# hyye/lio-mapping

Measured on NVIDIA H100. Metric: scans/sec + GN-iter ms, HDL-64 window=10 at 1/2/4/8 H100 vs CPU Ceres ref, higher is better.
Workload: dtype f32 features / f64 solve

## Files before the change

### include/lio_b200.h

```cpp
#ifndef LIO_B200_H_
#define LIO_B200_H_

#include <stddef.h>
#include <stdint.h>

#ifdef __cplusplus
extern "C" {
#endif

typedef enum lio_status {
  LIO_OK = 0,
  LIO_ERR_CUDA = -1,
  LIO_ERR_INVALID = -2,
  LIO_ERR_CAPACITY = -3,
  LIO_ERR_NO_DEVICE = -4,
  LIO_ERR_NUMERIC = -5
} lio_status;

const char *lio_last_error(void);
int lio_version(void);
int lio_device_count(void);

typedef struct lio_pp_config {
  float lower_bound;
// ... 190 lines not shown
int lio_est_set_scan_clouds_dev(lio_est *est, const float *corner_dev, const int *nc_dev, int nc_max, const float *full_dev,
                                const int *nf_dev, int nf_max);
int lio_est_local_clouds_dev(lio_est *est, const float *ptr[3], const int **n_dev, int n_host[3]);
int lio_est_local_clouds_download(lio_est *est, int which, float *out, int cap, int *n);
int lio_est_local_laser_odom(lio_est *est, float tf7[7]);
int lio_est_attach_map(lio_est *est, lio_pm *pm);
int lio_est_map_poses(lio_est *est, float tobe7[7], float aft7[7], float insert7[7], int info4[4]);
int lio_est_get_states(lio_est *est, double *out);
int lio_est_summary(lio_est *est, double *out32);
int lio_est_feature_count(lio_est *est, int frame, int *n);
int lio_est_get_features(lio_est *est, int frame, float *pts4, float *coef4, int32_t *src, int cap);
int lio_est_map_size(lio_est *est, int *n);
int lio_est_get_map(lio_est *est, float *out, int cap);
int lio_est_frame_size(lio_est *est, int frame, int *n);
int lio_est_get_frame(lio_est *est, int frame, float *out, int cap);
int lio_est_get_local_transform(lio_est *est, int frame, float tf7[7]);
int lio_est_prior_dim(lio_est *est, int *n);
int lio_est_get_prior(lio_est *est, double *Hp, double *bp);
int lio_est_last_normal_equations(lio_est *est, double *H, double *g, double *cost, int *n);
int lio_est_last_launches(lio_est *est);
const char *lio_est_last_error(lio_est *est);
int lio_est_solver_trace(lio_est *est, long long *out, int cap);
int lio_est_kernel_profile(lio_est *est, double out[8], int reset);
typedef int (*lio_allreduce_fn)(void *user, double *buf_dev, int count);
int lio_est_set_shard(lio_est *est, int rank, int world, lio_allreduce_fn fn, void *user);
int lio_est_exchange_buffer(lio_est *est, void **dev_ptr, size_t *bytes);
int lio_est_set_peers(lio_est *est, int world, void *const *peer_ptrs );
int lio_est_feature_slab(lio_est *est, void **dev_ptr, size_t *bytes);
int lio_est_set_feature_peers(lio_est *est, int world, void *const *peer_slabs );
int lio_ipc_export(const void *dev_ptr, unsigned char handle[64]);
int lio_ipc_open(const unsigned char handle[64], void **dev_ptr);
int lio_ipc_close(void *dev_ptr);
int lio_est_frame_owner(int frame_rel, int world);

int lio_compact_encode(const float tf7[7], const float *corner, int nc, const float *surf, int ns, const float *full, int nf,
                       float *out_xyzi, int cap_points, int *n_points);
int lio_compact_sizes(const float *xyzi, int n_points, int sizes[3]);
int lio_compact_decode(const float *xyzi, int n_points, float tf7[7], float *corner, float *surf, float *full);
int lio_xyzi_to_pcl32(const float *xyzi, int n, uint8_t *out32);
int lio_pcl32_to_xyzi(const uint8_t *in32, int n, float *xyzi);

int lio_host_cholesky_solve(int n, const double *A, const double *b, double *L_out, double *x);
int lio_host_sym_eigen(int n, const double *A, double *evals, double *evecs, int threads);
int lio_host_dogleg_toy(int n, int m, const double *A, const double *B, const double *y, double amp, int use_cauchy, double *x,
                        int max_iter, double *summary);

// ... 5 lines not shown
```

### lio_mapping_b200/_lib.py

```python
from __future__ import annotations

import ctypes as C
import os

import numpy as np

_HERE = os.path.dirname(os.path.abspath(__file__))
LIB_PATH = os.path.join(_HERE, "liblio_b200.so")
_LIB = None


class LioError(RuntimeError):
    pass


STATUS = {0: "LIO_OK", -1: "LIO_ERR_CUDA", -2: "LIO_ERR_INVALID", -3: "LIO_ERR_CAPACITY", -4: "LIO_ERR_NO_DEVICE",
          -5: "LIO_ERR_NUMERIC"}

f32p = np.ctypeslib.ndpointer(np.float32, flags="C_CONTIGUOUS")
f64p = np.ctypeslib.ndpointer(np.float64, flags="C_CONTIGUOUS")
i32p = np.ctypeslib.ndpointer(np.int32, flags="C_CONTIGUOUS")
u8p = np.ctypeslib.ndpointer(np.uint8, flags="C_CONTIGUOUS")
i8p = np.ctypeslib.ndpointer(np.int8, flags="C_CONTIGUOUS")

# ... 128 lines not shown
    L.lio_ipc_export.argtypes = [vp, u8p]
    L.lio_ipc_open.argtypes = [u8p, C.POINTER(vp)]
    L.lio_ipc_close.argtypes = [vp]
    L.lio_est_process_imu_batch.argtypes = [vp, ip, f64p, f64p, f64p, f64p]
    L.lio_est_process_scan_dev.argtypes = [vp, vp, vp, ip]
    L.lio_est_get_states.argtypes = [vp, f64p]
    L.lio_est_summary.argtypes = [vp, f64p]
    L.lio_est_feature_count.argtypes = [vp, ip, C.POINTER(ip)]
    L.lio_est_get_features.argtypes = [vp, ip, f32p, f32p, i32p, ip]
    L.lio_est_map_size.argtypes = [vp, C.POINTER(ip)]
    L.lio_est_get_map.argtypes = [vp, f32p, ip]
    L.lio_est_frame_size.argtypes = [vp, ip, C.POINTER(ip)]
    L.lio_est_get_frame.argtypes = [vp, ip, f32p, ip]
    L.lio_est_get_local_transform.argtypes = [vp, ip, f32p]
    L.lio_est_prior_dim.argtypes = [vp, C.POINTER(ip)]
    L.lio_est_get_prior.argtypes = [vp, f64p, f64p]
    L.lio_est_last_normal_equations.argtypes = [vp, f64p, f64p, C.POINTER(C.c_double), C.POINTER(ip)]
    L.lio_est_last_launches.argtypes = [vp]
    L.lio_est_last_error.argtypes = [vp]
    L.lio_est_last_error.restype = C.c_char_p
    L.lio_est_solver_trace.argtypes = [vp, np.ctypeslib.ndpointer(np.int64, flags="C_CONTIGUOUS"), ip]
    L.lio_est_frame_owner.argtypes = [ip, ip]
    L.lio_est_kernel_profile.argtypes = [vp, f64p, ip]
    L.lio_est_set_shard.argtypes = [vp, ip, ip, ALLREDUCE_FN, vp]
    L.lio_est_enable_local_clouds.argtypes = [vp, C.c_float, ip, ip]
    L.lio_est_set_scan_clouds_host.argtypes = [vp, f32p, ip, f32p, ip]
    L.lio_est_set_scan_clouds_dev.argtypes = [vp, vp, vp, ip, vp, vp, ip]
    L.lio_est_local_clouds_dev.argtypes = [vp, C.POINTER(vp), C.POINTER(vp), i32p]
    L.lio_est_local_clouds_download.argtypes = [vp, ip, f32p, ip, C.POINTER(ip)]
    L.lio_est_local_laser_odom.argtypes = [vp, f32p]
    L.lio_est_attach_map.argtypes = [vp, vp]
    L.lio_est_map_poses.argtypes = [vp, f32p, f32p, f32p, i32p]
    L.lio_mb_process_map_dev.argtypes = [vp, vp, vp, vp, vp, i32p, f32p, f32p, f32p, i32p]
    L.lio_po_process_dev.argtypes = [vp, C.POINTER(vp), C.POINTER(vp), i32p, f32p, f32p, i32p]
    L.lio_po_clouds_dev.argtypes = [vp, C.POINTER(vp), C.POINTER(vp), i32p]
    L.lio_pm_process_dev.argtypes = [vp, vp, vp, vp, vp, i32p, f32p, f32p, f32p, i32p]
    L.lio_pm_enable_publish.argtypes = [vp, C.c_float, ip]
    L.lio_pm_update_map_database_host.argtypes = [vp, f32p, ip, f32p, ip, np.ctypeslib.ndpointer(np.int64, flags="C_CONTIGUOUS"), ip,
                                                  f32p, i32p]
    L.lio_pm_update_stats.argtypes = [vp, i32p]
    _LIB = L
    return L


def check(rc: int, what: str = ""):
    if rc != 0:
# ... 10 lines not shown
```

### lio_mapping_b200/csrc/estimator.cu

```cuda
#include "assemble.cuh"
#include "cubemap.cuh"
#include <atomic>
#include <condition_variable>
#include <functional>
#include <mutex>
#include <thread>
#include "factors_host.h"
#include "factors_impl.h"
#include "knn.cuh"
#include "odom.cuh"
#include "qr.cuh"
#include "solver_dev.cuh"
#include "solver_host.h"
#include "voxel.cuh"
#include <chrono>
#include <cstddef>
#include <memory>
#include <new>
#include <vector>

namespace lio {
using namespace hm;

constexpr int kMaxWindow = 32;
// ... 269 lines not shown
      st->AtA[a * 6 + b] = v; st->AtA[b * 6 + a] = v;
    } else {
      st->AtB[threadIdx.x - 21] = v;
    }
  }
  __syncthreads();
  if (threadIdx.x == 0) odom_solve_step(st, tf_dev, delta_r_abort, delta_t_abort);
}

}

using namespace lio;
using namespace lio::hm;

struct lio_pim {
  std::shared_ptr<Preintegration> p;
};

struct ImuStampedF {
  double time;
  float q[4];
  float p[3];
};

struct MargPrior {
  bool valid = false;
  int n = 0;
  Mat Hp;
  Vec bp;
  double c0 = 0;
  std::vector<double> x0_pose, x0_sb;
  double x0_ex[7];
};

constexpr size_t kXRowBytes = sizeof(double) * kMaxOpt * kAsmStride;
constexpr size_t kXFlagOff = 2 * kXRowBytes;
constexpr size_t kXErrOff = kXFlagOff + sizeof(unsigned) * kMaxPeers;
constexpr size_t kXBytes = kXErrOff + 64;

struct MargJob {
  bool stashed = false, running = false;
  int O = 0;
  Mat A;
  Vec b;
  std::vector<double> x0_pose, x0_sb;
  double x0_ex[7];
// ... 172 lines not shown
  bool frames_started = false;
  float lc_corner_leaf = 0.2f;
  int lc_cap[2] = {0, 0};
  std::vector<float4 *> lc_slot[2];
  int *d_lc_slot_n = nullptr;
  float4 *d_lc_stage[2] = {nullptr, nullptr};
  int *d_lc_stage_n = nullptr;
  float4 *d_lc_pub[3] = {nullptr, nullptr, nullptr};
  int *d_lc_pub_n = nullptr;
  int lc_pub_cap[3] = {0, 0, 0};
  VoxelGrid lc_vg;
  cudaStream_t lc_stream = nullptr;
  cudaEvent_t lc_ev_fork = nullptr, lc_ev_join = nullptr;
  TransformF es{0, 0, 0, 1, 0, 0, 0};
  lio_pm *map = nullptr;
  bool scanned = false;
  int map_scans = 0;
  bool map_pending = false;
  float4 *d_keep[2] = {nullptr, nullptr};
  int *d_keep_n = nullptr;
  cudaEvent_t map_ev_in = nullptr, map_ev_done = nullptr;
  lio::TwistF map_insert;
  int map_info[4] = {0, 0, 0, 0};
};

static Tw tlb_double(const lio_est *e) {
  return Tw(Q(e->tlb_q[3], e->tlb_q[0], e->tlb_q[1], e->tlb_q[2]), V3(e->tlb_p[0], e->tlb_p[1], e->tlb_p[2]));
}

static Tw lidar_pose(const V3 &P, const M3 &R, const Tw &tlb) {
  Q rot = fromR(R * toR(inverse(tlb.rot)));
  V3 pos = P - rotate(rot, tlb.pos);
  return Tw(rot, pos);
}

struct AffineF { float R[9]; float t[3]; TransformF tf; };
static AffineF to_affine_f(const Tw &t) {
  AffineF a;
  float qx = (float)t.rot.x, qy = (float)t.rot.y, qz = (float)t.rot.z, qw = (float)t.rot.w;
  float n = std::sqrt(qx * qx + qy * qy + qz * qz + qw * qw);
  qx /= n; qy /= n; qz /= n; qw /= n;
  const float tx = 2.f * qx, ty = 2.f * qy, tz = 2.f * qz;
  const float twx = tx * qw, twy = ty * qw, twz = tz * qw, txx = tx * qx, txy = ty * qx, txz = tz * qx;
  const float tyy = ty * qy, tyz = tz * qy, tzz = tz * qz;
  a.R[0] = 1.f - (tyy + tzz); a.R[1] = txy - twz; a.R[2] = txz + twy;
  a.R[3] = txy + twz; a.R[4] = 1.f - (txx + tzz); a.R[5] = tyz - twx;
  a.R[6] = txz - twy; a.R[7] = tyz + twx; a.R[8] = 1.f - (txx + tyy);
// ... 108 lines not shown
  if (e->xbuf) cudaFree(e->xbuf);
  if (e->h_tf) cudaFreeHost(e->h_tf);
  if (e->h_S) cudaFreeHost(e->h_S);
  if (e->h_Rt) cudaFreeHost(e->h_Rt);
  if (e->d_Rt) cudaFree(e->d_Rt);
  if (e->h_counts) cudaFreeHost(e->h_counts);
  e->vg.destroy(); e->hash.destroy(); e->knn.destroy(); e->knn2.destroy(); e->asmw.destroy();
  if (e->ostream) cudaStreamDestroy(e->ostream);
  if (e->ev_map) cudaEventDestroy(e->ev_map);
  if (e->ev_odom) cudaEventDestroy(e->ev_odom);
  if (e->lc_stream) cudaStreamSynchronize(e->lc_stream);
  for (int w = 0; w < 2; ++w) {
    for (float4 *p : e->lc_slot[w]) if (p) cudaFree(p);
    if (e->d_lc_stage[w]) cudaFree(e->d_lc_stage[w]);
  }
  for (int w = 0; w < 3; ++w) if (e->d_lc_pub[w]) cudaFree(e->d_lc_pub[w]);
  if (e->d_lc_slot_n) cudaFree(e->d_lc_slot_n);
  if (e->d_lc_stage_n) cudaFree(e->d_lc_stage_n);
  if (e->d_lc_pub_n) cudaFree(e->d_lc_pub_n);
  e->lc_vg.destroy();
  if (e->lc_stream) cudaStreamDestroy(e->lc_stream);
  if (e->lc_ev_fork) cudaEventDestroy(e->lc_ev_fork);
  if (e->lc_ev_join) cudaEventDestroy(e->lc_ev_join);
  delete e;
  return LIO_OK;
}

extern "C" int lio_est_create(const lio_est_config *cfg, int device, void *cuda_stream, lio_est **out) {
  if (!cfg || !out) return LIO_ERR_INVALID;
  const int W = cfg->window_size, O = cfg->opt_window_size;
  if (W < 1 || W >= kMaxWindow || O < 1 || O > W || O > kMaxOpt || cfg->max_frame_points < 16 || cfg->max_scan_points < 16 ||
      !(cfg->surf_filter_size > 0) || !(cfg->min_match_sq_dis > 0) || cfg->odom_max_iterations < 1) {
    lio_set_last_error(__FILE__, __LINE__, "lio_est_create: configuration outside supported limits");
    return LIO_ERR_INVALID;
  }
  if (lio_device_count() <= 0) return LIO_ERR_NO_DEVICE;
  LIO_CUDA_OK(cudaSetDevice(device));
  lio_est *e = new (std::nothrow) lio_est();
  if (!e) return LIO_ERR_INVALID;
  e->cfg = *cfg; e->W = W; e->O = O; e->device = device; e->stream = (cudaStream_t)cuda_stream;
  cudaDeviceGetAttribute(&e->sm_count, cudaDevAttrMultiProcessorCount, device);
  e->noise.acc_n = cfg->acc_n; e->noise.gyr_n = cfg->gyr_n; e->noise.acc_w = cfg->acc_w; e->noise.gyr_w = cfg->gyr_w; e->noise.g_norm = cfg->g_norm;
  e->g_vec = V3(0, 0, -cfg->g_norm);
  e->extrinsic_stage = cfg->estimate_extrinsic;
  e->Ps.assign(W + 1, V3()); e->Vs.assign(W + 1, V3()); e->Bas.assign(W + 1, V3()); e->Bgs.assign(W + 1, V3());
  e->Rs.assign(W + 1, M3::I());
// ... 15 lines not shown
  }
  e->local_cap = e->slot_cap + cfg->max_frame_points * (O > 1 ? O - 1 : 1);
  ok = ok && cudaMalloc(&e->d_slot_n, sizeof(int) * (W + 1)) == cudaSuccess;
  ok = ok && cudaMalloc(&e->d_own_n, sizeof(int) * (W + 1)) == cudaSuccess;
  ok = ok && cudaMalloc(&e->d_scan, sizeof(float4) * cfg->max_scan_points) == cudaSuccess;
  ok = ok && cudaMalloc(&e->d_local, sizeof(float4) * e->local_cap) == cudaSuccess;
  ok = ok && cudaMalloc(&e->d_map, sizeof(float4) * e->local_cap) == cudaSuccess;
  ok = ok && cudaMalloc(&e->d_tmp, sizeof(float4) * e->slot_cap) == cudaSuccess;
  ok = ok && cudaMalloc(&e->d_counts, sizeof(int) * 8) == cudaSuccess;
  ok = ok && cudaMalloc(&e->d_tf, sizeof(TransformF) * (W + 1)) == cudaSuccess;
  ok = ok && cudaMalloc(&e->d_odom, sizeof(OdomState)) == cudaSuccess;
  ok = ok && cudaMalloc(&e->d_odom_partial, sizeof(double) * 32 * 1024) == cudaSuccess;
  ok = ok && cudaMallocHost((void **)&e->h_tf, sizeof(TransformF) * (W + 1)) == cudaSuccess;
  ok = ok && cudaMallocHost((void **)&e->h_S, sizeof(double) * kMaxOpt * kAsmStride) == cudaSuccess;
  ok = ok && cudaMallocHost((void **)&e->h_Rt, sizeof(double) * kMaxOpt * kAsmRtStride) == cudaSuccess;
  ok = ok && cudaMalloc(&e->d_Rt, sizeof(double) * kMaxOpt * kAsmRtStride) == cudaSuccess;
  ok = ok && cudaMallocHost((void **)&e->h_counts, sizeof(int) * (W + 16)) == cudaSuccess;
  if (ok) { std::memset(e->h_counts, 0, sizeof(int) * (W + 16)); e->h_xerr = e->h_counts + W + 10; }
  int vg_cap = std::max(e->local_cap, cfg->max_scan_points);
  ok = ok && e->vg.init(vg_cap) == 0;
  ok = ok && e->hash.init(e->local_cap) == 0;
  ok = ok && e->knn.init(cfg->max_frame_points * (O + 1)) == 0;
  ok = ok && e->knn2.init(cfg->max_frame_points) == 0;
  ok = ok && cudaStreamCreateWithFlags(&e->ostream, cudaStreamNonBlocking) == cudaSuccess;
  ok = ok && cudaEventCreateWithFlags(&e->ev_map, cudaEventDisableTiming) == cudaSuccess;
  ok = ok && cudaEventCreateWithFlags(&e->ev_odom, cudaEventDisableTiming) == cudaSuccess;
  e->feats.assign(W + 1, FeatureOut());
  long long total_feat = 0;
  {
    e->foff_pts.assign(W + 1, 0); e->foff_coef.assign(W + 1, 0);
    size_t off = 0;
    for (int k = pivot + 1; k <= W; ++k) {
      const int cap = cfg->max_frame_points * ((k == W && cfg->keep_features) ? cfg->odom_max_iterations : 1);
      e->feats[k].cap = cap;
      e->foff_pts[k] = off; off += sizeof(float4) * (size_t)cap;
      e->foff_coef[k] = off; off += sizeof(float4) * (size_t)cap;
      total_feat += cap;
    }
    e->foff_cnt = off; off += ((sizeof(int) * (size_t)(W + 1) + 255) / 256) * 256;
    e->fpar_stride = off;
    e->foff_flags = 2 * off;
    e->fslab_bytes = 2 * off + 256;
    ok = ok && cudaMalloc(&e->fslab, e->fslab_bytes) == cudaSuccess && cudaMemset(e->fslab, 0, e->fslab_bytes) == cudaSuccess;
    for (int k = pivot + 1; k <= W && ok; ++k) ok = ok && cudaMalloc(&e->feats[k].src, sizeof(int) * e->feats[k].cap) == cudaSuccess;
    if (ok) set_feature_parity(e, 0);
  }
  ok = ok && e->asmw.init((int)std::min<long long>(total_feat, 1ll << 30)) == 0;
// ... 342 lines not shown
  for (int i = 0; i <= W; ++i) {
    AffineF a = to_affine_f(tw_mul(pivot_inv, lidar_pose(e->Ps[i], e->Rs[i], tlb)));
    e->local_tf[i] = a.tf;
    e->h_tf[i] = a.tf;
    if (i < pivot || i == W) continue;
    cp.src[ns] = e->slot_ptr[e->slot_of[i]];
    cp.n[ns] = e->d_slot_n + e->slot_of[i];
    if (i == pivot) cp.identity[ns] = 1;
    else { std::memcpy(cp.R[ns], a.R, sizeof(a.R)); std::memcpy(cp.t[ns], a.t, sizeof(a.t)); cp.tag[ns] = (float)i; }
    ++ns;
  }
  cp.nsrc = ns;
  EST_CUDA(cudaMemcpyAsync(e->d_tf, e->h_tf, sizeof(TransformF) * (W + 1), cudaMemcpyHostToDevice, st));
  k_concat<<<std::max(1, std::min(e->sm_count * 4, (e->local_cap + 255) / 256)), 256, 0, st>>>(cp, e->d_local, e->d_counts + 1, e->local_cap);
  ++e->launches;
  long long bound = 64;
  for (int i = 0; i < W; ++i) bound += e->size_surf_stack[i] > 0 ? e->size_surf_stack[i] : e->cfg.max_frame_points;
  const int n_bound = (int)std::min<long long>(e->local_cap, bound);
  int rc = e->vg.run(e->d_local, e->d_counts + 1, n_bound, e->cfg.surf_filter_size, e->d_map, e->local_cap, e->d_counts + 2, nullptr, st, &e->launches);
  if (rc != LIO_OK) return rc;
  const float cell = std::sqrt(e->cfg.min_match_sq_dis) * (1.0f + 1.0f / 1024.0f);
  rc = e->hash.build(e->d_map, e->d_counts + 2, n_bound, cell, st, &e->launches);
  if (rc != LIO_OK) return rc;
  e->t_build = now_s() - t0;
  const double t1 = now_s();
  if (e->fpeers) {
    set_feature_parity(e, e->fparity ^ 1);
    ++e->fepoch;
    for (int idx = pivot + 1; idx <= W; ++idx)
      if (owns_frame(e, idx)) EST_CUDA(cudaMemsetAsync(e->d_feat_counts + idx, 0, sizeof(int), st));
  } else {
    EST_CUDA(cudaMemsetAsync(e->d_feat_counts, 0, sizeof(int) * (W + 1), st));
  }
  constexpr int kOdomFirstBatch = 3;
  const bool odom = e->cfg.imu_factor && owns_frame(e, W);
  KnnBatch ob;
  auto odom_rounds = [&](int from, int to, cudaStream_t q) -> int {
    const int idx = W, slot = e->slot_of[W];
    if (!e->cfg.keep_features) {
      ob.nframes = 1;
      KnnFrame &f = ob.f[0];
      f.surf = e->slot_ptr[slot]; f.n_dev = e->d_slot_n + slot; f.n_bound = e->cfg.max_frame_points; f.tf = e->d_tf + idx;
      f.out_p = e->feats[idx].pts; f.out_c = e->feats[idx].coef; f.out_src = e->feats[idx].src; f.out_count = e->feats[idx].count;
      f.append = 0; f.tile0 = 0;
      for (int it = from; it < to; ++it) {
        int r2 = calculate_features_batch(e->hash, ob, e->cfg.min_match_sq_dis, e->cfg.min_plane_dis, &e->d_odom->done, e->knn2, q, &e->launches,
// ... 26 lines not shown
    rc = odom_rounds(0, odom_first, e->ostream);
    if (rc != LIO_OK) return rc;
    EST_CUDA(cudaEventRecord(e->ev_odom, e->ostream));
  }
  {
    KnnBatch b;
    b.nframes = 0;
    for (int idx = pivot + 1; idx <= W; ++idx) {
      if (!owns_frame(e, idx)) continue;
      if (idx == W && e->cfg.imu_factor) continue;
      const int slot = e->slot_of[idx];
      KnnFrame &f = b.f[b.nframes++];
      f.surf = e->slot_ptr[slot]; f.n_dev = e->d_slot_n + slot; f.tf = e->d_tf + idx;
      const int known = e->size_surf_stack[idx];
      f.n_bound = (known > 0 && idx < W) ? known : e->cfg.max_frame_points;
      f.out_p = e->feats[idx].pts; f.out_c = e->feats[idx].coef; f.out_src = e->feats[idx].src; f.out_count = e->feats[idx].count;
      f.append = 0; f.tile0 = 0;
    }
    e->knn_timed = b.nframes > 0 && e->evk0 && e->evk1;
    if (e->knn_timed) cudaEventRecord(e->evk0, st);
    rc = calculate_features_batch(e->hash, b, e->cfg.min_match_sq_dis, e->cfg.min_plane_dis, nullptr, e->knn, st, &e->launches);
    if (rc != LIO_OK) return rc;
    if (e->knn_timed) cudaEventRecord(e->evk1, st);
  }
  auto readback = [&]() -> int {
    EST_CUDA(cudaMemcpyAsync(e->h_counts, e->d_feat_counts, sizeof(int) * (W + 1), cudaMemcpyDeviceToHost, st));
    EST_CUDA(cudaMemcpyAsync(e->h_counts + W + 1, e->d_counts, sizeof(int) * 4, cudaMemcpyDeviceToHost, st));
    EST_CUDA(cudaMemcpyAsync(e->h_counts + W + 5, &e->d_odom->iter, sizeof(int), cudaMemcpyDeviceToHost, st));
    EST_CUDA(cudaMemcpyAsync(e->h_tf + W, e->d_tf + W, sizeof(TransformF), cudaMemcpyDeviceToHost, st));
    EST_CUDA(cudaMemcpyAsync(e->h_counts + W + 6, e->d_slot_n + e->slot_of[W], sizeof(int), cudaMemcpyDeviceToHost, st));
    EST_CUDA(cudaMemcpyAsync(e->h_counts + W + 7, e->vg.overflow_flag(), sizeof(int), cudaMemcpyDeviceToHost, st));
    EST_CUDA(cudaMemcpyAsync(e->h_counts + W + 8, &e->d_odom->done, sizeof(int), cudaMemcpyDeviceToHost, st));
    if (e->fpeers) EST_CUDA(cudaMemcpyAsync(e->h_counts + W + 9, e->fslab + e->foff_flags + 128, sizeof(int), cudaMemcpyDeviceToHost, st));
    if (e->map) EST_CUDA(cudaMemcpyAsync(e->h_counts + W + 13, e->d_lc_stage_n + 1, sizeof(int), cudaMemcpyDeviceToHost, st));
    EST_CUDA(cudaStreamSynchronize(st));
    return LIO_OK;
  };
  if (odom) EST_CUDA(cudaStreamWaitEvent(st, e->ev_odom, 0));
  if (e->fpeers) {
    const size_t pbase = (size_t)e->fparity * e->fpar_stride;
    FeaturePeers fp;
    std::memset(&fp, 0, sizeof(fp));
    fp.npeers = e->world; fp.self = e->rank;
    FlagPeers fl;
    std::memset(&fl, 0, sizeof(fl));
    fl.npeers = e->world; fl.self = e->rank;
    for (int r = 0; r < e->world; ++r) fl.flag[r] = reinterpret_cast<unsigned *>(e->fpeer_base[r] + e->foff_flags);
    for (int idx = pivot + 1; idx <= W; ++idx) {
      if (!owns_frame(e, idx)) continue;
      for (int r = 0; r < e->world; ++r) {
        fp.pts[r] = reinterpret_cast<float4 *>(e->fpeer_base[r] + pbase + e->foff_pts[idx]);
        fp.coef[r] = reinterpret_cast<float4 *>(e->fpeer_base[r] + pbase + e->foff_coef[idx]);
        fp.count[r] = reinterpret_cast<int *>(e->fpeer_base[r] + pbase + e->foff_cnt) + idx;
      }
      const int known = e->size_surf_stack[idx];
      const int bound = (known > 0 && idx < W) ? known : e->feats[idx].cap;
      k_publish_features<<<std::max(1, std::min(e->sm_count * 2, (bound + 255) / 256)), 256, 0, st>>>(e->feats[idx].pts, e->feats[idx].coef, e->feats[idx].count,
                                                                                                   e->feats[idx].cap, fp);
      ++e->launches;
    }
    k_publish_flag<<<1, 32, 0, st>>>(fl, e->fepoch);
    k_xwait<<<1, 32, 0, st>>>(reinterpret_cast<const unsigned *>(e->fslab + e->foff_flags), e->world, e->fepoch,
                              reinterpret_cast<int *>(e->fslab + e->foff_flags + 128), nullptr);
    e->launches += 2;
  }
  if (before_sync) {
    rc = before_sync();
    if (rc != LIO_OK) return rc;
  }
  rc = readback();
  if (rc != LIO_OK) return rc;
  if (odom && odom_first < odom_total && !e->h_counts[W + 8]) {
    rc = odom_rounds(odom_first, odom_total, st);
    if (rc != LIO_OK) return rc;
    rc = readback();
    if (rc != LIO_OK) return rc;
  }
  if (e->fpeers && (rc = xwait_report(e, Exchange::features, st)) != LIO_OK) return rc;
  if (e->h_counts[W + 6] > e->cfg.max_frame_points) {
    lio_set_last_error(__FILE__, __LINE__, "down-sampled scan exceeds max_frame_points");
    return LIO_ERR_CAPACITY;
  }
  if (e->h_counts[W + 7]) {
    cudaMemsetAsync(e->vg.overflow_flag(), 0, sizeof(int), st);
    lio_set_last_error(__FILE__, __LINE__, "voxel grid index overflow (leaf size too small for the cloud extent)");
    return LIO_ERR_CAPACITY;
  }
  e->size_surf_stack[W] = e->h_counts[W + 6];
  if (e->knn_timed) {
    float ms = 0.f;
    if (cudaEventElapsedTime(&ms, e->evk0, e->evk1) == cudaSuccess) {
      long long nq = 0;
      for (int idx = pivot + 1; idx <= W; ++idx)
        if (owns_frame(e, idx) && !(idx == W && e->cfg.imu_factor)) nq += e->size_surf_stack[idx];
      e->knn_ms_sum += ms; e->knn_launch_count += 1; e->knn_query_sum += nq;
    }
  }
  for (int k = 0; k <= W; ++k) e->h_feat_n[k] = e->h_counts[k];
  e->h_map_n = e->h_counts[W + 1 + 2];
  e->odom_iters = e->h_counts[W + 5];
// ... 303 lines not shown
      add_lidar_block(S, ft[i].M, &H, &g, off_pose(0), off_pose(i), oe);
    }
    e->t_lin_lidar += now_s() - tl0;
  }
  cost = cp + ci + cm + cprior;
  if (c_pim) *c_pim = ci;
  if (c_ppp) *c_ppp = cp;
  if (c_marg) *c_marg = cm;
  return std::isfinite(cost) ? LIO_OK : LIO_ERR_NUMERIC;
}

static void prior_join(lio_est *e);
static int solve_dev_prepare(lio_est *e, int max_it, bool assemble_only);
static int slide_window(lio_est *e);
static MargPrior marg_algebra(Mat A, Vec b, int O, std::vector<double> x0_pose, std::vector<double> x0_sb, const double *x0_ex);
static int marginalize(lio_est *e) {
  const int O = e->O, pivot = e->W - O;
  const int m = 15, nr = 15 * O + 6, pos = m + nr;
  Mat A(pos, pos);
  Vec b(pos, 0.0);
  auto idx_pose = [&](int k) { return k == 0 ? 0 : m + 15 * (k - 1); };
  auto idx_sb = [&](int k) { return k == 0 ? 6 : m + 15 * (k - 1) + 6; };
  const int idx_ex = m + 15 * O;
  if (e->prior.valid) {
    const MargPrior &pr = e->prior;
    Vec dx;
    prior_dx(e, pr, dx);
    Vec Hdx;
    matvec(pr.Hp, dx, Hdx);
    auto map = [&](int pi) {
      if (pi >= 15 * O) return idx_ex + (pi - 15 * O);
      int k = pi / 15, a = pi % 15;
      return (a < 6 ? idx_pose(k) + a : idx_sb(k) + (a - 6));
    };
    for (int a = 0; a < pr.n; ++a) {
      const int ia = map(a);
      b[ia] += Hdx[a] + pr.bp[a];
      for (int c = 0; c < pr.n; ++c) A(ia, map(c)) += pr.Hp(a, c);
    }
  }
  if (e->cfg.imu_factor && e->pre[pivot + 1]->sum_dt < 10.0) {
    double r[15], J[15][30];
    imu_factor_evaluate30(*e->pre[pivot + 1], e->para_pose[0].data(), e->para_sb[0].data(), e->para_pose[1].data(), e->para_sb[1].data(), r, J);
    int col[30];
    for (int c = 0; c < 6; ++c) { col[c] = idx_pose(0) + c; col[15 + c] = idx_pose(1) + c; }
    for (int c = 0; c < 9; ++c) { col[6 + c] = idx_sb(0) + c; col[21 + c] = idx_sb(1) + c; }
    add_JtJ_mapped(&J[0][0], r, 15, 30, col, A, b);
  }
  if (e->cfg.point_distance_factor) {
    std::vector<FrameTerms> ft;
    int rc = eval_lidar(e, ft);
    if (rc != LIO_OK) return rc;
    for (int i = 1; i <= O; ++i) add_lidar_block(e->h_S + (i - 1) * kAsmStride, ft[i].M, &A, &b, idx_pose(0), idx_pose(i), idx_ex);
  }
  MargJob &job = e->mjob;
  job.O = O;
  job.A.r = A.r; job.A.c = A.c; job.A.d.swap(A.d);
  job.b.swap(b);
  job.x0_pose.resize(7 * O); job.x0_sb.resize(9 * O);
  for (int k = 1; k <= O; ++k) {
    std::memcpy(&job.x0_pose[7 * (k - 1)], e->para_pose[k].data(), 7 * sizeof(double));
    std::memcpy(&job.x0_sb[9 * (k - 1)], e->para_sb[k].data(), 9 * sizeof(double));
  }
  std::memcpy(job.x0_ex, e->para_ex, sizeof(job.x0_ex));
  job.stashed = true;
  if (!e->cfg.overlap_marginalization) {
    job.stashed = false;
    e->prior = marg_algebra(std::move(job.A), std::move(job.b), job.O, std::move(job.x0_pose), std::move(job.x0_sb), job.x0_ex);
    e->hp_exp_valid = false;
  }
  return LIO_OK;
}

static MargPrior marg_algebra(Mat A, Vec b, int O, std::vector<double> x0_pose, std::vector<double> x0_sb, const double *x0_ex) {
  const int m = 15, nr = 15 * O + 6;
  const double eps = 1e-8;
  Mat Amm(m, m);
  for (int r = 0; r < m; ++r) for (int c = 0; c < m; ++c) Amm(r, c) = 0.5 * (A(r, c) + A(c, r));
  Vec ev;
  Mat evec;
  sym_eigen(Amm, ev, evec);
  Mat Amm_inv(m, m);
  for (int r = 0; r < m; ++r)
    for (int c = 0; c < m; ++c) { double s = 0; for (int k = 0; k < m; ++k) s += evec(r, k) * (ev[k] > eps ? 1.0 / ev[k] : 0.0) * evec(c, k); Amm_inv(r, c) = s; }
  Mat Tm(nr, m);
  for (int r = 0; r < nr; ++r) for (int c = 0; c < m; ++c) { double s = 0; for (int k = 0; k < m; ++k) s += A(m + r, k) * Amm_inv(k, c); Tm(r, c) = s; }
  Mat A2(nr, nr);
  Vec b2(nr);
  for (int r = 0; r < nr; ++r) {
    for (int c = 0; c < nr; ++c) { double s = 0; for (int k = 0; k < m; ++k) s += Tm(r, k) * A(k, m + c); A2(r, c) = A(m + r, m + c) - s; }
    double s = 0;
    for (int k = 0; k < m; ++k) s += Tm(r, k) * b[k];
    b2[r] = b[m + r] - s;
  }
  std::vector<int> nz;
  for (int r = 0; r < nr; ++r) {
    bool any = b2[r] != 0.0;
    const double *row = &A2.d[(size_t)r * nr];
    for (int c = 0; c < nr && !any; ++c) any = row[c] != 0.0 || A2.d[(size_t)c * nr + r] != 0.0;
    if (any) nz.push_back(r);
  }
  const int nc = (int)nz.size();
  Mat Ac(nc, nc);
  Vec bc(nc);
  for (int r = 0; r < nc; ++r) {
    bc[r] = b2[nz[r]];
    for (int c = 0; c < nc; ++c) Ac(r, c) = A2(nz[r], nz[c]);
  }
  Vec ev2;
  Mat V2;
  if (nc > 0) sym_eigen(Ac, ev2, V2, 1);
  MargPrior np;
  np.valid = true;
// ... 107 lines not shown
      for (int a = 0; a < 9; ++a) out[16 * k + 7 + a] = x[16 * k + 7 + a] + d[15 * k + 6 + a];
    }
    if (ex_free) pose_plus(&x[16 * (O + 1)], &d[15 * (O + 1)], &out[16 * (O + 1)]);
  };
  DoglegOptions opt;
  opt.max_num_iterations = max_it;
  dogleg_solve(opt, P, &e->summary);
  if (eval_rc != LIO_OK) return eval_rc;
  if (e->summary.termination == 2 && !std::isfinite(e->summary.final_cost)) { lio_set_last_error(__FILE__, __LINE__, "solver breakdown"); return LIO_ERR_NUMERIC; }
  e->t_solve = now_s() - t0;
  return LIO_OK;
}

static int map_step(lio_est *e);
static int scan_close_window(lio_est *e) {
  double_to_vector(e);
  const double t1 = now_s();
  if (e->cfg.marginalization_factor && !e->turn_off) {
    vector_to_double(e);
    const int rc = marginalize(e);
    if (rc != LIO_OK) return rc;
    e->prior_uploaded = false;
  }
  e->t_marg = now_s() - t1;
  e->window_open = false;
  int rc = lc_join(e);
  if (rc != LIO_OK) return rc;
  if (e->map && (rc = map_step(e)) != LIO_OK) return rc;
  return slide_window(e);
}

static int solve_dev_prepare(lio_est *e, int max_it, bool assemble_only) {
  const int O = e->O, pivot = e->W - O;
  cudaStream_t st = e->stream;
  DevSolveState &S = *e->ds.h_st;
  S.sc.O = O; S.sc.n = 15 * (O + 1) + 6; S.sc.max_it = assemble_only ? 0 : max_it;
  S.sc.skip_gates = assemble_only ? 1 : 0; S.sc.pad_ = 0;
  S.sc.imu_factor = e->cfg.imu_factor; S.sc.point_distance_factor = e->cfg.point_distance_factor;
  S.sc.prior_factor = e->cfg.prior_factor; S.sc.marginalization_factor = e->cfg.marginalization_factor;
  S.sc.ex_free = e->ex_constant ? 0 : 1;
  S.sc.prior_valid = (e->cfg.marginalization_factor && e->prior.valid) ? 1 : 0;
  S.sc.convergence_flag = e->convergence_flag ? 1 : 0;
  S.sc.turn_off = 1; S.sc.done = 0; S.sc.iteration = 0; S.sc.successful = 0; S.sc.evaluations = 0; S.sc.termination = 0; S.sc.reuse = 0; S.sc.invalid = 0;
  for (int k = 0; k <= O; ++k) { std::memcpy(S.x + 16 * k, e->para_pose[k].data(), 7 * sizeof(double)); std::memcpy(S.x + 16 * k + 7, e->para_sb[k].data(), 9 * sizeof(double)); }
  std::memcpy(S.x + 16 * (O + 1), e->para_ex, 7 * sizeof(double));
  {
// ... 271 lines not shown
  if (!e->tmp_pre) { lio_set_last_error(__FILE__, __LINE__, "process_scan before finish_init"); return LIO_ERR_INVALID; }
  if (e->lc_on && !e->lc_staged) {
    lio_set_last_error(__FILE__, __LINE__, "local clouds are on: stage the scan's corner / full cloud with lio_est_set_scan_clouds_* first");
    std::snprintf(e->err, sizeof(e->err), "%s", lio_last_error());
    return LIO_ERR_INVALID;
  }
  e->frames_started = true;
  e->scanned = true;
  const int rc = process_scan_body(e, scan_dev, n_dev, n_max, open_only);
  if (rc != LIO_OK) { e->poisoned = true; std::snprintf(e->err, sizeof(e->err), "%s", lio_last_error()); }
  return rc;
}

static int map_scan_entry(lio_est *e);
static int process_scan_body(lio_est *e, const float4 *scan_dev, const int *n_dev, int n_max, bool open_only) {
  const int W = e->W;
  cudaStream_t st = e->stream;
  marg_start(e);
  const double t0 = now_s();
  e->launches = 0;
  e->t_lin_wait = e->t_lin_host = e->t_lin_lidar = e->t_marg_wait = 0;
  e->have_H0 = false;
  if (!e->tmp_pre) { lio_set_last_error(__FILE__, __LINE__, "process_scan before finish_init"); return LIO_ERR_INVALID; }
  if (e->map) {
    const int rc0 = map_scan_entry(e);
    if (rc0 != LIO_OK) return rc0;
  }
  push_shift(e->pre, e->tmp_pre);
  e->tmp_pre = std::make_shared<Preintegration>(e->acc_last, e->gyr_last, e->Bas[W], e->Bgs[W], e->noise);
  {
    const int freed = e->slot_of[0];
    e->slot_of.erase(e->slot_of.begin());
    e->slot_of.push_back(freed);
  }
  const int slot = e->slot_of[W];
  const float4 *src = scan_dev;
  const bool es_on = (e->cfg.enable_deskew || e->cfg.cutoff_deskew) && !e->imu_stamped.empty();
  const bool deskew_surf = es_on && !e->cfg.cutoff_deskew;
  if (es_on) {
    const ImuStampedF &te = e->imu_stamped.back();
    ImuStampedF ts = te;
    for (int i = (int)e->imu_stamped.size() - 1; i >= 0; --i) {
      ts = e->imu_stamped[i];
      if (te.time - e->imu_stamped[i].time >= 0.1) break;
    }
    auto twf = [](const float *q, const float *p) { return Tw(Q(q[3], q[0], q[1], q[2]), V3(p[0], p[1], p[2])); };
// ... 3 lines not shown
      Q qe = body_es.rot;
      double d = qe.w, absD = std::fabs(d), s0, s1;
      if (absD >= 1.0 - 1.1920929e-7) { s0 = 1.0 - s; s1 = s; }
      else { double th = std::acos(absD), sn = std::sin(th); s0 = std::sin((1.0 - s) * th) / sn; s1 = std::sin(s * th) / sn; }
      if (d < 0) s1 = -s1;
      body_es.rot = Q(s0 + s1 * qe.w, s1 * qe.x, s1 * qe.y, s1 * qe.z);
      body_es.pos = body_es.pos * (double)s;
    }
    const Tw tlb = tlb_double(e);
    const Tw es = tw_mul(tw_mul(tlb, body_es), tw_inverse(tlb));
    e->es = TransformF{(float)es.rot.x, (float)es.rot.y, (float)es.rot.z, (float)es.rot.w, (float)es.pos.x, (float)es.pos.y, (float)es.pos.z};
  }
  if (deskew_surf) {
    if (scan_dev != e->d_scan) {
      EST_CUDA(cudaMemcpyAsync(e->d_scan, scan_dev, sizeof(float4) * n_max, cudaMemcpyDeviceToDevice, st));
    }
    k_deskew<<<(n_max + 255) / 256, 256, 0, st>>>(e->d_scan, n_dev, e->es, 10.f);
    ++e->launches;
    src = e->d_scan;
  }
  int rc = e->vg.run(src, n_dev, n_max, e->cfg.surf_filter_size, e->slot_ptr[slot], e->cfg.max_frame_points, e->d_slot_n + slot, nullptr, st, &e->launches);
  if (rc != LIO_OK) return rc;
  EST_CUDA(cudaMemcpyAsync(e->d_own_n + slot, e->d_slot_n + slot, sizeof(int), cudaMemcpyDeviceToDevice, st));
  if (e->lc_on && (rc = lc_push(e, deskew_surf)) != LIO_OK) return rc;
  push_shift(e->size_surf_stack, 0);
  rc = scan_open_window(e);
  if (rc != LIO_OK || open_only) return rc;
  rc = scan_solve(e, e->cfg.max_num_iterations);
  if (rc != LIO_OK) return rc;
  rc = scan_close_window(e);
  if (rc != LIO_OK) return rc;
  e->t_total = now_s() - t0;
  return LIO_OK;
}

extern "C" int lio_est_begin_scan(lio_est *e) {
  if (!e) return LIO_ERR_INVALID;
  if (e->cfg.overlap_marginalization) marg_start(e);
  return LIO_OK;
}

extern "C" int lio_est_process_scan_host(lio_est *e, const float *surf_last, int n) {
  if (!e || n < 0 || (n > 0 && !surf_last)) return LIO_ERR_INVALID;
  if (n > e->cfg.max_scan_points) return LIO_ERR_CAPACITY;
  LIO_CUDA_OK(cudaSetDevice(e->device));
  if (n > 0) LIO_CUDA_OK(cudaMemcpyAsync(e->d_scan, surf_last, sizeof(float4) * n, cudaMemcpyHostToDevice, e->stream));
  e->h_counts[e->W + 8] = n;
  LIO_CUDA_OK(cudaMemcpyAsync(e->d_counts, e->h_counts + e->W + 8, sizeof(int), cudaMemcpyHostToDevice, e->stream));
  return process_scan_common(e, e->d_scan, e->d_counts, n > 0 ? n : 1);
}

extern "C" int lio_est_process_scan_dev(lio_est *e, const float *surf_last_dev, const int *n_dev, int n_max) {
  if (!e || !surf_last_dev || !n_dev || n_max <= 0) return LIO_ERR_INVALID;
  if (n_max > e->cfg.max_scan_points) n_max = e->cfg.max_scan_points;
// ... 322 lines not shown
    LIO_CUDA_OK(cudaSetDevice(e->device));
    std::vector<double> Hf((size_t)nf * nf), gf(nf);
    LIO_CUDA_OK(cudaMemcpy(Hf.data(), e->ds.H0, sizeof(double) * nf * nf, cudaMemcpyDeviceToHost));
    LIO_CUDA_OK(cudaMemcpy(gf.data(), e->ds.g0, sizeof(double) * nf, cudaMemcpyDeviceToHost));
    if (H) for (int r = 0; r < nr; ++r) std::memcpy(H + (size_t)r * nr, &Hf[(size_t)r * nf], sizeof(double) * nr);
    if (g) std::memcpy(g, gf.data(), sizeof(double) * nr);
    if (cost) *cost = e->cost0;
    return LIO_OK;
  }
  *n = e->H0.r;
  if (H) std::memcpy(H, e->H0.d.data(), sizeof(double) * e->H0.r * e->H0.r);
  if (g) std::memcpy(g, e->g0.data(), sizeof(double) * e->H0.r);
  if (cost) *cost = e->cost0;
  return LIO_OK;
}
extern "C" int lio_est_last_launches(lio_est *e) { return e ? e->launches : 0; }
extern "C" const char *lio_est_last_error(lio_est *e) { return e ? e->err : "null handle"; }

extern "C" int lio_est_solver_trace(lio_est *e, long long *out, int cap) {
  if (!e || !out || cap < 24 * 16 + 4 * 28 + 4) return LIO_ERR_INVALID;
  if (!e->use_dev_solver) { std::memset(out, 0, sizeof(long long) * (24 * 16 + 4 * 28 + 4)); return LIO_OK; }
  LIO_CUDA_OK(cudaSetDevice(e->device));
  LIO_CUDA_OK(cudaMemcpy(out, reinterpret_cast<const char *>(e->ds.st) + offsetof(DevSolveState, dbg), sizeof(long long) * (24 * 16 + 4 * 28 + 4), cudaMemcpyDeviceToHost));
  return LIO_OK;
}

extern "C" int lio_est_kernel_profile(lio_est *e, double out[8], int reset) {
  if (!e || !out) return LIO_ERR_INVALID;
  out[0] = e->asm_ms_sum; out[1] = (double)e->asm_launch_count; out[2] = (double)e->asm_feat_sum; out[3] = 32.0;
  out[4] = e->knn_ms_sum; out[5] = (double)e->knn_launch_count; out[6] = (double)e->knn_query_sum; out[7] = 128.0;
  if (reset) { e->asm_ms_sum = 0; e->asm_launch_count = 0; e->asm_feat_sum = 0; e->knn_ms_sum = 0; e->knn_launch_count = 0; e->knn_query_sum = 0; }
  return LIO_OK;
}

extern "C" int lio_ppp_evaluate(const double point[3], const double coeff[4], const double pose_pivot[7], const double pose_i[7],
                                const double pose_ex[7], double *residual, double *J0, double *J1, double *J2) {
  if (!point || !coeff || !pose_pivot || !pose_i || !pose_ex || !residual) return LIO_ERR_INVALID;
  ppp_evaluate_single(point, coeff, pose_pivot, pose_i, pose_ex, residual, J0, J1, J2);
  return LIO_OK;
}

namespace lio {
int ppp_rows_launch(const float4 *pts, const float4 *coef, int n, const double *Rt12_dev, const double *M_dev, double *r_out,
                    double *J_out, cudaStream_t st);
}

// ... 415 lines not shown
```

### lio_mapping_b200/estimator.py

```python
from __future__ import annotations

import ctypes as C

import numpy as np

from . import _lib

SUMMARY_KEYS = ["iterations", "successful", "termination", "initial_cost", "final_cost", "cost_pim", "cost_ppp", "cost_marg",
                "turn_off", "convergence_flag", "map_size", "num_features", "odom_iters", "t_build_map", "t_features",
                "t_solve", "t_marg", "t_total", "has_prior", "linearizations", "cost_evals", "launches", "t_lin_wait", "t_lin_host",
                "t_lin_lidar", "t_marg_wait"]


def _d(a):
    return np.ascontiguousarray(a, np.float64)


def ppp_evaluate(point, coeff, pose_pivot, pose_i, pose_ex):
    r = np.zeros(1)
    J = [np.zeros(7) for _ in range(3)]
    _lib.check(_lib.lib().lio_ppp_evaluate(_d(point), _d(coeff), _d(pose_pivot), _d(pose_i), _d(pose_ex), r, J[0], J[1], J[2]),
               "lio_ppp_evaluate")
    return float(r[0]), J

# ... 203 lines not shown
        _lib.check(_lib.lib().lio_est_set_feature_peers(self.h, world, arr), "lio_est_set_feature_peers")

    @staticmethod
    def _peer_array(rank, world, own, ptrs, handles, opened):
        arr = (C.c_void_p * world)()
        for r in range(world):
            if r == rank:
                arr[r] = own
            elif ptrs is not None:
                arr[r] = int(ptrs[r])
            else:
                p = C.c_void_p()
                _lib.check(_lib.lib().lio_ipc_open(np.ascontiguousarray(handles[r], np.uint8), C.byref(p)), "lio_ipc_open")
                opened.append(p.value)
                arr[r] = p.value
        return arr

    def kernel_profile(self, reset=False):
        o = np.zeros(8)
        _lib.check(_lib.lib().lio_est_kernel_profile(self.h, o, 1 if reset else 0), "kernel_profile")
        return dict(asm_ms=o[0], asm_launches=int(o[1]), asm_features=int(o[2]), bytes_per_feature=o[3],
                    knn_ms=o[4], knn_launches=int(o[5]), knn_queries=int(o[6]), bytes_per_query=o[7])

    def solver_trace(self):
        out = np.zeros(24 * 16 + 4 * 28 + 4, np.int64)
        _lib.check(_lib.lib().lio_est_solver_trace(self.h, out, out.size), "lio_est_solver_trace")
        self.chol_profile = out[24 * 16:]
        return out[:24 * 16].reshape(24, 16)

    def states(self):
        out = np.zeros((self.W + 1, 16))
        _lib.check(_lib.lib().lio_est_get_states(self.h, out), "lio_est_get_states")
        return out

    def local_laser_odom(self):
        t = np.zeros(7, np.float32)
        _lib.check(_lib.lib().lio_est_local_laser_odom(self.h, t), "lio_est_local_laser_odom")
        return t

    LOCAL_CLOUDS = ("corner", "surf", "full")

    def enable_local_clouds(self, corner_filter_size=0.2, max_corner_points=1 << 16, max_full_points=1 << 18):
        _lib.check(_lib.lib().lio_est_enable_local_clouds(self.h, float(corner_filter_size), int(max_corner_points), int(max_full_points)),
                   "lio_est_enable_local_clouds")

    def set_scan_clouds(self, corner, full):
# ... 84 lines not shown
```

Baseline: 434.2.

## Add phase timing events, prioritize odom stream, overlap lidar eval, speed host marg

Adds optional CUDA-event phase timing with a Python API. It also creates the odometry stream at the highest priority, launches the lidar factor evaluation before the host adds the prior so the two overlap, and precomputes the prior index map with row-pointer accumulation. The Schur complement product is reordered into a cache-friendly row-accumulate loop. Together these aim to cut host-side marginalization cost and GPU/host serialization, at the cost of mixing unrelated changes and adding timing instrumentation.

```diff
diff --git a/include/lio_b200.h b/include/lio_b200.h
--- a/include/lio_b200.h
+++ b/include/lio_b200.h
@@ -236,6 +236,8 @@
 const char *lio_est_last_error(lio_est *est);
 int lio_est_solver_trace(lio_est *est, long long *out, int cap);
 int lio_est_kernel_profile(lio_est *est, double out[8], int reset);
+int lio_est_phase_timing(lio_est *est, int on);
+int lio_est_phase_times(lio_est *est, void *ref_event, float *out_ms, int cap);
 typedef int (*lio_allreduce_fn)(void *user, double *buf_dev, int count);
 int lio_est_set_shard(lio_est *est, int rank, int world, lio_allreduce_fn fn, void *user);
 int lio_est_exchange_buffer(lio_est *est, void **dev_ptr, size_t *bytes);
diff --git a/lio_mapping_b200/_lib.py b/lio_mapping_b200/_lib.py
--- a/lio_mapping_b200/_lib.py
+++ b/lio_mapping_b200/_lib.py
@@ -174,6 +174,8 @@
     L.lio_est_solver_trace.argtypes = [vp, np.ctypeslib.ndpointer(np.int64, flags="C_CONTIGUOUS"), ip]
     L.lio_est_frame_owner.argtypes = [ip, ip]
     L.lio_est_kernel_profile.argtypes = [vp, f64p, ip]
+    L.lio_est_phase_timing.argtypes = [vp, ip]
+    L.lio_est_phase_times.argtypes = [vp, vp, f32p, ip]
     L.lio_est_set_shard.argtypes = [vp, ip, ip, ALLREDUCE_FN, vp]
     L.lio_est_enable_local_clouds.argtypes = [vp, C.c_float, ip, ip]
     L.lio_est_set_scan_clouds_host.argtypes = [vp, f32p, ip, f32p, ip]
diff --git a/lio_mapping_b200/csrc/estimator.cu b/lio_mapping_b200/csrc/estimator.cu
--- a/lio_mapping_b200/csrc/estimator.cu
+++ b/lio_mapping_b200/csrc/estimator.cu
@@ -315,6 +315,8 @@
   float q[4];
   float p[3];
 };
+
+enum { kPhEntry, kPhFrameVg, kPhLocalMap, kPhKnn, kPhOdom, kPhReadback, kPhSolve, kPhMarg, kPhSlide, kPhases };
 
 struct MargPrior {
   bool valid = false;
@@ -533,7 +535,13 @@
   cudaEvent_t map_ev_in = nullptr, map_ev_done = nullptr;
   lio::TwistF map_insert;
   int map_info[4] = {0, 0, 0, 0};
+  cudaEvent_t ph_ev[kPhases] = {};
+  bool ph_on = false;
 };
+
+static void phase_mark(lio_est *e, int k, cudaStream_t q) {
+  if (e->ph_on) cudaEventRecord(e->ph_ev[k], q);
+}
 
 static Tw tlb_double(const lio_est *e) {
   return Tw(Q(e->tlb_q[3], e->tlb_q[0], e->tlb_q[1], e->tlb_q[2]), V3(e->tlb_p[0], e->tlb_p[1], e->tlb_p[2]));
@@ -688,6 +696,7 @@
   if (e->lc_stream) cudaStreamDestroy(e->lc_stream);
   if (e->lc_ev_fork) cudaEventDestroy(e->lc_ev_fork);
   if (e->lc_ev_join) cudaEventDestroy(e->lc_ev_join);
+  for (cudaEvent_t ev : e->ph_ev) if (ev) cudaEventDestroy(ev);
   delete e;
   return LIO_OK;
 }
@@ -749,7 +758,11 @@
   ok = ok && e->hash.init(e->local_cap) == 0;
   ok = ok && e->knn.init(cfg->max_frame_points * (O + 1)) == 0;
   ok = ok && e->knn2.init(cfg->max_frame_points) == 0;
-  ok = ok && cudaStreamCreateWithFlags(&e->ostream, cudaStreamNonBlocking) == cudaSuccess;
+  {
+    int prio_least = 0, prio_greatest = 0;
+    ok = ok && cudaDeviceGetStreamPriorityRange(&prio_least, &prio_greatest) == cudaSuccess;
+    ok = ok && cudaStreamCreateWithPriority(&e->ostream, cudaStreamNonBlocking, prio_greatest) == cudaSuccess;
+  }
   ok = ok && cudaEventCreateWithFlags(&e->ev_map, cudaEventDisableTiming) == cudaSuccess;
   ok = ok && cudaEventCreateWithFlags(&e->ev_odom, cudaEventDisableTiming) == cudaSuccess;
   e->feats.assign(W + 1, FeatureOut());
@@ -1138,6 +1151,7 @@
   const float cell = std::sqrt(e->cfg.min_match_sq_dis) * (1.0f + 1.0f / 1024.0f);
   rc = e->hash.build(e->d_map, e->d_counts + 2, n_bound, cell, st, &e->launches);
   if (rc != LIO_OK) return rc;
+  phase_mark(e, kPhLocalMap, st);
   e->t_build = now_s() - t0;
   const double t1 = now_s();
   if (e->fpeers) {
@@ -1210,6 +1224,7 @@
     rc = calculate_features_batch(e->hash, b, e->cfg.min_match_sq_dis, e->cfg.min_plane_dis, nullptr, e->knn, st, &e->launches);
     if (rc != LIO_OK) return rc;
     if (e->knn_timed) cudaEventRecord(e->evk1, st);
+    phase_mark(e, kPhKnn, st);
   }
   auto readback = [&]() -> int {
     EST_CUDA(cudaMemcpyAsync(e->h_counts, e->d_feat_counts, sizeof(int) * (W + 1), cudaMemcpyDeviceToHost, st));
@@ -1225,6 +1240,7 @@
     return LIO_OK;
   };
   if (odom) EST_CUDA(cudaStreamWaitEvent(st, e->ev_odom, 0));
+  phase_mark(e, kPhOdom, st);
   if (e->fpeers) {
     const size_t pbase = (size_t)e->fparity * e->fpar_stride;
     FeaturePeers fp;
@@ -1264,6 +1280,7 @@
     rc = readback();
     if (rc != LIO_OK) return rc;
   }
+  phase_mark(e, kPhReadback, st);
   if (e->fpeers && (rc = xwait_report(e, Exchange::features, st)) != LIO_OK) return rc;
   if (e->h_counts[W + 6] > e->cfg.max_frame_points) {
     lio_set_last_error(__FILE__, __LINE__, "down-sampled scan exceeds max_frame_points");
@@ -1613,21 +1630,28 @@
   auto idx_pose = [&](int k) { return k == 0 ? 0 : m + 15 * (k - 1); };
   auto idx_sb = [&](int k) { return k == 0 ? 6 : m + 15 * (k - 1) + 6; };
   const int idx_ex = m + 15 * O;
+  std::vector<FrameTerms> ft;
+  if (e->cfg.point_distance_factor) {
+    int rc = eval_lidar_launch(e, ft);
+    if (rc != LIO_OK) return rc;
+  }
   if (e->prior.valid) {
     const MargPrior &pr = e->prior;
     Vec dx;
     prior_dx(e, pr, dx);
     Vec Hdx;
     matvec(pr.Hp, dx, Hdx);
-    auto map = [&](int pi) {
-      if (pi >= 15 * O) return idx_ex + (pi - 15 * O);
-      int k = pi / 15, a = pi % 15;
-      return (a < 6 ? idx_pose(k) + a : idx_sb(k) + (a - 6));
-    };
+    std::vector<int> map(pr.n);
+    for (int pi = 0; pi < pr.n; ++pi) {
+      const int k = pi / 15, a = pi % 15;
+      map[pi] = pi >= 15 * O ? idx_ex + (pi - 15 * O) : (a < 6 ? idx_pose(k) + a : idx_sb(k) + (a - 6));
+    }
     for (int a = 0; a < pr.n; ++a) {
-      const int ia = map(a);
+      const int ia = map[a];
       b[ia] += Hdx[a] + pr.bp[a];
-      for (int c = 0; c < pr.n; ++c) A(ia, map(c)) += pr.Hp(a, c);
+      const double *hrow = &pr.Hp.d[(size_t)a * pr.n];
+      double *arow = &A.d[(size_t)ia * pos];
+      for (int c = 0; c < pr.n; ++c) arow[map[c]] += hrow[c];
     }
   }
   if (e->cfg.imu_factor && e->pre[pivot + 1]->sum_dt < 10.0) {
@@ -1639,8 +1663,7 @@
     add_JtJ_mapped(&J[0][0], r, 15, 30, col, A, b);
   }
   if (e->cfg.point_distance_factor) {
-    std::vector<FrameTerms> ft;
-    int rc = eval_lidar(e, ft);
+    int rc = eval_lidar_wait(e);
     if (rc != LIO_OK) return rc;
     for (int i = 1; i <= O; ++i) add_lidar_block(e->h_S + (i - 1) * kAsmStride, ft[i].M, &A, &b, idx_pose(0), idx_pose(i), idx_ex);
   }
@@ -1678,8 +1701,16 @@
   for (int r = 0; r < nr; ++r) for (int c = 0; c < m; ++c) { double s = 0; for (int k = 0; k < m; ++k) s += A(m + r, k) * Amm_inv(k, c); Tm(r, c) = s; }
   Mat A2(nr, nr);
   Vec b2(nr);
+  Vec acc(nr);
   for (int r = 0; r < nr; ++r) {
-    for (int c = 0; c < nr; ++c) { double s = 0; for (int k = 0; k < m; ++k) s += Tm(r, k) * A(k, m + c); A2(r, c) = A(m + r, m + c) - s; }
+    std::fill(acc.begin(), acc.end(), 0.0);
+    for (int k = 0; k < m; ++k) {
+      const double t = Tm(r, k);
+      const double *arow = &A.d[(size_t)k * A.c + m];
+      for (int c = 0; c < nr; ++c) acc[c] += t * arow[c];
+    }
+    const double *keep = &A.d[(size_t)(m + r) * A.c + m];
+    for (int c = 0; c < nr; ++c) A2(r, c) = keep[c] - acc[c];
     double s = 0;
     for (int k = 0; k < m; ++k) s += Tm(r, k) * b[k];
     b2[r] = b[m + r] - s;
@@ -1833,6 +1864,7 @@
     if (rc != LIO_OK) return rc;
     e->prior_uploaded = false;
   }
+  phase_mark(e, kPhMarg, e->stream);
   e->t_marg = now_s() - t1;
   e->window_open = false;
   int rc = lc_join(e);
@@ -2150,6 +2182,7 @@
   e->t_lin_wait = e->t_lin_host = e->t_lin_lidar = e->t_marg_wait = 0;
   e->have_H0 = false;
   if (!e->tmp_pre) { lio_set_last_error(__FILE__, __LINE__, "process_scan before finish_init"); return LIO_ERR_INVALID; }
+  phase_mark(e, kPhEntry, st);
   if (e->map) {
     const int rc0 = map_scan_entry(e);
     if (rc0 != LIO_OK) return rc0;
@@ -2199,14 +2232,17 @@
   int rc = e->vg.run(src, n_dev, n_max, e->cfg.surf_filter_size, e->slot_ptr[slot], e->cfg.max_frame_points, e->d_slot_n + slot, nullptr, st, &e->launches);
   if (rc != LIO_OK) return rc;
   EST_CUDA(cudaMemcpyAsync(e->d_own_n + slot, e->d_slot_n + slot, sizeof(int), cudaMemcpyDeviceToDevice, st));
+  phase_mark(e, kPhFrameVg, st);
   if (e->lc_on && (rc = lc_push(e, deskew_surf)) != LIO_OK) return rc;
   push_shift(e->size_surf_stack, 0);
   rc = scan_open_window(e);
   if (rc != LIO_OK || open_only) return rc;
   rc = scan_solve(e, e->cfg.max_num_iterations);
   if (rc != LIO_OK) return rc;
+  phase_mark(e, kPhSolve, st);
   rc = scan_close_window(e);
   if (rc != LIO_OK) return rc;
+  phase_mark(e, kPhSlide, st);
   e->t_total = now_s() - t0;
   return LIO_OK;
 }
@@ -2575,6 +2611,21 @@
   if (!e->use_dev_solver) { std::memset(out, 0, sizeof(long long) * (24 * 16 + 4 * 28 + 4)); return LIO_OK; }
   LIO_CUDA_OK(cudaSetDevice(e->device));
   LIO_CUDA_OK(cudaMemcpy(out, reinterpret_cast<const char *>(e->ds.st) + offsetof(DevSolveState, dbg), sizeof(long long) * (24 * 16 + 4 * 28 + 4), cudaMemcpyDeviceToHost));
+  return LIO_OK;
+}
+
+extern "C" int lio_est_phase_timing(lio_est *e, int on) {
+  if (!e) return LIO_ERR_INVALID;
+  LIO_CUDA_OK(cudaSetDevice(e->device));
+  for (cudaEvent_t &ev : e->ph_ev) if (on && !ev) LIO_CUDA_OK(cudaEventCreate(&ev));
+  e->ph_on = on != 0;
+  return LIO_OK;
+}
+
+extern "C" int lio_est_phase_times(lio_est *e, void *ref_event, float *out_ms, int cap) {
+  if (!e || !ref_event || !out_ms || cap < kPhases || !e->ph_on) return LIO_ERR_INVALID;
+  LIO_CUDA_OK(cudaSetDevice(e->device));
+  for (int k = 0; k < kPhases; ++k) LIO_CUDA_OK(cudaEventElapsedTime(&out_ms[k], (cudaEvent_t)ref_event, e->ph_ev[k]));
   return LIO_OK;
 }
 
diff --git a/lio_mapping_b200/estimator.py b/lio_mapping_b200/estimator.py
--- a/lio_mapping_b200/estimator.py
+++ b/lio_mapping_b200/estimator.py
@@ -249,6 +249,17 @@
         return dict(asm_ms=o[0], asm_launches=int(o[1]), asm_features=int(o[2]), bytes_per_feature=o[3],
                     knn_ms=o[4], knn_launches=int(o[5]), knn_queries=int(o[6]), bytes_per_query=o[7])
 
+    PHASES = ("entry", "frame_voxel_grid", "local_map_hash", "batched_knn", "odom_joined", "readback", "solve", "marginalize",
+              "slide_window")
+
+    def phase_timing(self, on=True):
+        _lib.check(_lib.lib().lio_est_phase_timing(self.h, 1 if on else 0), "lio_est_phase_timing")
+
+    def phase_times(self, ref_event):
+        out = np.zeros(len(self.PHASES), np.float32)
+        _lib.check(_lib.lib().lio_est_phase_times(self.h, C.c_void_p(ref_event.cuda_event), out, out.size), "lio_est_phase_times")
+        return dict(zip(self.PHASES, out.tolist()))
+
     def solver_trace(self):
         out = np.zeros(24 * 16 + 4 * 28 + 4, np.int64)
         _lib.check(_lib.lib().lio_est_solver_trace(self.h, out, out.size), "lio_est_solver_trace")
```

Measured after the change: 441.7, median of 6. No clear change (+1.7%).
